# google/deepconsensus

Measured on AMD Instinct MI355X. Metric: zmw_per_sec, higher is better.
Workload: dtype bf16; 1 GPU; global_batch=16384, seq_len=100, windows_per_zmw=150, parallelism=dp1, native_kernels=True, hipgraph=True

## Files before the change

deepconsensus_amd/models/runner.py:

```python
from __future__ import annotations

import copy
import math
from typing import List, Optional, Tuple

import torch

from deepconsensus_amd import ops as dc_ops
from deepconsensus_amd.calibration.calibration import (
    parse_calibration_string,
)
from deepconsensus_amd.models.config import Params
from deepconsensus_amd.models.model import (
    EncoderOnlyLearnedValuesTransformer,
    get_model,
)
from deepconsensus_amd.utils import constants
from deepconsensus_amd.utils import trace


def build_gather_tables(model: EncoderOnlyLearnedValuesTransformer):
    (bi, pwi, ipi, sti, ci, bqi, sni) = model.indices

    def scaled(emb):
        t = emb.table.detach().float() * math.sqrt(emb.width)
        t = t.clone()
        t[0].zero_()
        return t.to(torch.bfloat16)

    tables = {
        "bases": scaled(model.bases_embedding),
        "pw": scaled(model.pw_embedding),
        "ip": scaled(model.ip_embedding),
        "strand": scaled(model.strand_embedding),
        "sn": scaled(model.sn_embedding),
    }
    if model.use_ccs_bq:
        tables["ccs_bq"] = scaled(model.ccs_bq_embedding)

    order = ["bases", "pw", "ip", "strand", "sn"]
    if model.use_ccs_bq:
        order.append("ccs_bq")
    flat_parts, table_base = [], {}
    off = 0
    for name in order:
        t = tables[name]
        table_base[name] = off
        flat = t.reshape(-1)
        pad = (-flat.numel()) % 8
        if pad:
            flat = torch.cat([flat, flat.new_zeros(pad)])
        flat_parts.append(flat)
        off += flat.numel()
    table_flat = torch.cat(flat_parts).contiguous()

    plan: List[Tuple[str, int]] = []
    plan += [("bases", 0)] * (bi[1] - bi[0])
    plan += [("pw", 0)] * (pwi[1] - pwi[0])
    plan += [("ip", 0)] * (ipi[1] - ipi[0])
    plan += [("strand", 0)] * (sti[1] - sti[0])
    plan += [("bases", 0)] * (ci[1] - ci[0])
    if model.use_ccs_bq:
        plan += [("ccs_bq", 1)]
    plan += [("sn", 0)] * (sni[1] - sni[0])

    row_shift = torch.tensor([s for _, s in plan], dtype=torch.int32)
    row_vocab = torch.tensor(
        [tables[n].shape[0] for n, _ in plan], dtype=torch.int32
    )

    cols: List[Tuple[int, int, int]] = []
    for r, (name, _) in enumerate(plan):
        w = tables[name].shape[1]
        base = table_base[name]
        for j in range(w):
            cols.append((r, base, w))
    concat = len(cols)
    assert concat % 8 == 0, f"concat width {concat} not 8-aligned"
    nchunk = concat // 8
    chunk_cnt = torch.zeros(nchunk, dtype=torch.int32)
    chunk_entries = torch.zeros(nchunk * 4, 4, dtype=torch.int32)
    for c in range(nchunk):
        entries = []
        j = c * 8
        while j < (c + 1) * 8:
            r, base, w = cols[j]
            entries.append((r, base, w))
            j += w
        assert len(entries) <= 4, "chunk spans >4 table rows"
        if len(entries) == 1:
            assert entries[0][2] == 8, (
                f"chunk {c}: single entry must be width 8, got "
                f"{entries[0][2]} (row layout misaligned)"
            )
        else:
            assert all(w == 2 for _, _, w in entries), (
                f"chunk {c}: multi-entry chunk must be all width-2 "
                f"entries, got {[w for _, _, w in entries]}"
            )
        chunk_cnt[c] = len(entries)
        for k, (r, base, w) in enumerate(entries):
            chunk_entries[c * 4 + k] = torch.tensor([r, base, w, 0])
    return table_flat, row_shift, row_vocab, chunk_cnt, chunk_entries.reshape(-1)


_CONDENSE_WIDTHS = (560, 568, 872, 880)


def condense_image_stride(k: int) -> Optional[int]:
    if k not in _CONDENSE_WIDTHS:
        return None
    return 16 * (-(-k // 16)) + 8


def build_condense_image(weight: torch.Tensor) -> torch.Tensor:
    n, k = weight.shape
    ws = condense_image_stride(k)
    if ws is None:
        raise ValueError(
            f"fused_condense supports widths {_CONDENSE_WIDTHS}, got {k}"
        )
    npad = -(-n // 64) * 64
    img = torch.zeros(npad, ws, dtype=torch.bfloat16)
    img[:n, :k] = weight.detach().to(torch.bfloat16)
    return img.contiguous()


def fused_condense_enabled(k: int, value: Optional[str]) -> bool:
    if value == "0":
        return False
    if value == "wide":
        return condense_image_stride(k) is not None
    return k == 560


class InferenceRunner:

    def __init__(
        self,
        params: Params,
        model: Optional[torch.nn.Module] = None,
        device: Optional[str] = None,
        calibration: str = "skip",
        max_qual: int = constants.MAX_QUAL,
    ):
        self.params = params
        if device is None:
            device = "cuda" if torch.cuda.is_available() else "cpu"
        self.device = torch.device(device)
        self.calib = parse_calibration_string(calibration)
        self.max_qual = max_qual
        if model is None:
            model = get_model(params)
        model.eval()
        self.model = model

        self.native = (
            self.device.type == "cuda"
            and isinstance(model, EncoderOnlyLearnedValuesTransformer)
            and model.condense
        )
        if self.device.type == "cuda":
            self.ext = dc_ops.get_ext(required=self.native)
        else:
            self.ext = None

        self.model = model.to(self.device)
        if self.native:
            self._prepare_native(model)

    def _prepare_native(self, model) -> None:
        dev, bf16 = self.device, torch.bfloat16
        tf, rs, rv, cc, ce = build_gather_tables(model)
        self.table_flat = tf.to(dev)
        self.row_shift = rs.to(dev)
        self.row_vocab = rv.to(dev)
        self.chunk_cnt = cc.to(dev)
        self.chunk_entries = ce.to(dev)
        self.win = model.params.get("attn_win_size")
        self.num_heads = model.params["num_heads"]
        self.cond_wt = (
            model.condenser.weight.detach().t().contiguous().to(bf16).to(dev)
        )
        self.pos = (
            model.pos_encoding.to(bf16).to(dev)
            if model.add_pos_encoding
            else None
        )
        import os as _os

        self.cond_img = None
        self.pos_f32 = None
        cw = model.condenser.weight.detach()
        if fused_condense_enabled(
            cw.shape[1], _os.environ.get("DC_FUSED_CONDENSE")
        ):
            self.cond_img = build_condense_image(cw).to(dev)
            if model.add_pos_encoding:
                self.pos_f32 = (
                    model.pos_encoding.detach().float().contiguous().to(dev)
                )
        self.fused_embed = _os.environ.get("DC_FUSED_EMBED") != "0"
        self.rezero_fast = all(
            l.attn_wrap.rezero and l.ffn_wrap.rezero for l in model.layers
        ) and self.win is not None
        if self.rezero_fast:
            self.layer_w = []
            for l in model.layers:
                wq = l.attn.q_proj.weight.detach()
                wk = l.attn.k_proj.weight.detach()
                wv = l.attn.v_proj.weight.detach()
                wqkv_t = (
                    torch.cat([wq, wk, wv], 0).t().contiguous().to(bf16).to(dev)
                )
                self.layer_w.append(
                    dict(
                        wqkv_t=wqkv_t,
                        wout_t=l.attn.out_proj.weight.detach()
                        .t().contiguous().to(bf16).to(dev),
                        w1_t=l.ffn.filter_layer.weight.detach()
                        .t().contiguous().to(bf16).to(dev),
                        b1=l.ffn.filter_layer.bias.detach().to(bf16).to(dev),
                        w2_t=l.ffn.output_layer.weight.detach()
                        .t().contiguous().to(bf16).to(dev),
                        b2=l.ffn.output_layer.bias.detach().to(bf16).to(dev),
                        alpha_attn=float(l.attn_wrap.alpha.detach()),
                        alpha_ffn=float(l.ffn_wrap.alpha.detach()),
                    )
                )
            for lw in self.layer_w:
                lw["wout_t_a"] = lw["wout_t"] * lw["alpha_attn"]
                lw["w2_t_a"] = lw["w2_t"] * lw["alpha_ffn"]
                lw["b2_a"] = lw["b2"] * lw["alpha_ffn"]
            import os as _os

            self.ffn_fused_ok = (
                model.params["hidden_size"] == 280
                and model.params["filter_size"] == 2048
                and _os.environ.get("DC_FUSED_FFN") != "0"
            )
            self.ffn_v2 = _os.environ.get("DC_FFN_V2", "1") != "0"
            self.ffn_v3 = _os.environ.get("DC_FFN_V3", "1") != "0"
            self.ffn_v5 = _os.environ.get("DC_FFN_V5", "1") != "0"

            if self.ffn_fused_ok:
                for i, l in enumerate(model.layers):
                    lw = self.layer_w[i]
                    wq = l.attn.q_proj.weight.detach().float()
                    wk = l.attn.k_proj.weight.detach().float()
                    wv = l.attn.v_proj.weight.detach().float()
                    wqkv = torch.cat([wq, wk, wv], 0)
                    wqkv_pad = torch.zeros(896, 296)
                    wqkv_pad[:840, :280] = wqkv
                    lw["wqkv_pad"] = wqkv_pad.to(bf16).contiguous().to(dev)
                    wo = l.attn.out_proj.weight.detach().float()
                    wout_pad = torch.zeros(320, 296)
                    wout_pad[:280, :280] = wo
                    lw["wout_pad"] = wout_pad.to(bf16).contiguous().to(dev)
                    w1 = l.ffn.filter_layer.weight.detach().float()
                    w1p = torch.zeros(2048, 288)
                    w1p[:, :280] = w1
                    lw["w1_pad"] = w1p.to(bf16).contiguous().to(dev)
                    lw["b1_f32"] = (
                        l.ffn.filter_layer.bias.detach().float().to(dev)
                    )
                    w2 = l.ffn.output_layer.weight.detach().float()
                    w2p = torch.zeros(320, 2048)
                    w2p[:280] = w2
                    lw["w2_pad"] = w2p.to(bf16).contiguous().to(dev)
                    b2p = torch.zeros(320)
                    b2p[:280] = l.ffn.output_layer.bias.detach().float()
                    lw["b2_f32"] = b2p.to(dev)
                    w1v2 = torch.zeros(2048, 296)
                    w1v2[:, :280] = w1
                    w1v2[:, 287] = l.ffn.filter_layer.bias.detach().float()
                    lw["w1_v2"] = w1v2.to(bf16).contiguous().to(dev)
            self._addmm_act = hasattr(torch, "_addmm_activation")
            if self._addmm_act:
                try:
                    torch._addmm_activation(
                        torch.zeros(4, device=dev, dtype=bf16),
                        torch.zeros(2, 4, device=dev, dtype=bf16),
                        torch.zeros(4, 4, device=dev, dtype=bf16),
                    )
                except Exception:
                    self._addmm_act = False
        else:
            layers = copy.deepcopy(model.layers).to(bf16)
            for m in layers.modules():
                if isinstance(m, torch.nn.LayerNorm):
                    m.float()
            self.layers_bf16 = layers.to(dev)
        self.ln_gamma = model.output_norm.weight.detach().float().to(dev)
        self.ln_beta = model.output_norm.bias.detach().float().to(dev)
        self.w_head = model.fc1.weight.detach().float().contiguous().to(dev)
        self.b_head = model.fc1.bias.detach().float().to(dev)

    def _attn(self, qkv: torch.Tensor) -> torch.Tensor:
        b, l, w = qkv.shape
        d = w // (3 * self.num_heads)
        if d == 140 and 32 <= l <= 104 and 1 <= self.win <= 12:
            return self.ext.banded_attn_mfma(
                qkv, self.num_heads, self.win, d ** -0.5
            )
        return self.ext.banded_attn(qkv, self.num_heads, self.win)

    @torch.no_grad()
    def encode_native(self, rows: torch.Tensor) -> torch.Tensor:
        rows = rows.contiguous()
        b, _, l = rows.shape
        gather_args = (
            rows, self.table_flat, self.row_shift, self.row_vocab,
            self.chunk_cnt, self.chunk_entries,
        )
        if self.cond_img is not None:
            h = self.cond_wt.shape[1]
            pos = (
                self.pos_f32
                if self.pos_f32 is not None
                else torch.empty(0, dtype=torch.float32, device=rows.device)
            )
            if self.fused_embed:
                with trace.range("K2_K3_embed_condense"):
                    x = self.ext.fused_embed_condense(
                        *gather_args, self.cond_img, pos, h
                    )
            else:
                with trace.range("K2_embed_gather"):
                    emb = self.ext.embed_gather(*gather_args)
                with trace.range("K3_condenser"):
                    x = self.ext.fused_condense(
                        emb.reshape(b * l, -1), self.cond_img, pos, h, l
                    )
            x = x.view(b, l, -1)
        else:
            with trace.range("K2_embed_gather"):
                emb = self.ext.embed_gather(*gather_args)
            with trace.range("K3_condenser"):
                x = emb.reshape(b * l, -1) @ self.cond_wt
            x = x.view(b, l, -1)
            if self.pos is not None:
                x = x + self.pos[:l]
        if self.rezero_fast:
            h = x.shape[-1]
            flat = x.reshape(b * l, h)
            empty = flat.new_empty(0)
            for lw in self.layer_w:
                with trace.range("K5_qkv_proj"):
                    if self.ffn_fused_ok:
                        qkv = self.ext.fused_linear(
                            flat, lw["wqkv_pad"], empty, empty, 840,
                            False, 0.0
                        ).view(b, l, -1)
                    else:
                        qkv = (flat @ lw["wqkv_t"]).view(b, l, -1)
                with trace.range("K6_banded_attn"):
                    a = self._attn(qkv)
                if self.ffn_fused_ok:
                    with trace.range("K7_out_proj"):
                        flat = self.ext.fused_linear(
                            a.view(b * l, h), lw["wout_pad"], empty, flat,
                            280, False, lw["alpha_attn"],
                        )
                    with trace.range("K9_fused_ffn"):
                        if self.ffn_v5:
                            flat = self.ext.fused_ffn_v5(
                                flat, lw["w1_v2"], lw["w2_pad"],
                                lw["b2_f32"], lw["alpha_ffn"],
                            )
                        elif self.ffn_v3:
                            flat = self.ext.fused_ffn_v3(
                                flat, lw["w1_v2"], lw["w2_pad"],
                                lw["b2_f32"], lw["alpha_ffn"],
                            )
                        elif self.ffn_v2:
                            flat = self.ext.fused_ffn_v2(
                                flat, lw["w1_v2"], lw["w2_pad"],
                                lw["b2_f32"], lw["alpha_ffn"],
                            )
                        else:
                            flat = self.ext.fused_ffn(
                                flat, lw["w1_pad"], lw["b1_f32"],
                                lw["w2_pad"], lw["b2_f32"],
                                lw["alpha_ffn"],
                            )
                    continue
                flat = torch.addmm(flat, a.view(b * l, h), lw["wout_t_a"])
                if self._addmm_act:
                    ff = torch._addmm_activation(lw["b1"], flat, lw["w1_t"])
                    flat = torch.addmm(flat, ff, lw["w2_t_a"]).add_(lw["b2_a"])
                else:
                    ff = torch.addmm(lw["b1"], flat, lw["w1_t"]).relu_()
                    flat = torch.addmm(flat, ff, lw["w2_t_a"]).add_(lw["b2_a"])
            x = flat.view(b, l, h)
        else:
            for layer in self.layers_bf16:
                x, _ = layer(x, training=False)
        return x

    @torch.no_grad()
    def forward_windows_graphed(self, host_rows: torch.Tensor):
        if not self.native:
            return self.forward_windows(host_rows)
        shape = tuple(host_rows.shape)
        if getattr(self, "_graph_shape", None) != shape:
            try:
                g_in = torch.empty(
                    shape, dtype=host_rows.dtype, device=self.device
                )
                side = torch.cuda.Stream()
                side.wait_stream(torch.cuda.current_stream())
                with torch.cuda.stream(side):
                    for _ in range(2):
                        self.forward_windows(g_in)
                torch.cuda.current_stream().wait_stream(side)
                torch.cuda.synchronize()
                graph = torch.cuda.CUDAGraph()
                with torch.cuda.graph(graph):
                    g_bases, g_quals = self.forward_windows(g_in)
                torch.cuda.synchronize()
                self._graph = graph
                self._graph_in = g_in
                self._graph_out = (g_bases, g_quals)
                self._graph_shape = shape
            except Exception:
                self._graph_shape = None
                self._graph = None
                return self.forward_windows(host_rows)
        self._graph_in.copy_(host_rows, non_blocking=True)
        self._graph.replay()
        return self._graph_out

    @torch.no_grad()
    def forward_windows(
        self, rows: torch.Tensor, want_probs: bool = False
    ):
        rows = rows.to(self.device, non_blocking=True)
        if self.native:
            x = self.encode_native(rows)
            with trace.range("K10_K12_ln_head_qv"):
                out = self.ext.fused_ln_head_qv(
                x.reshape(-1, x.shape[-1]),
                self.ln_gamma,
                self.ln_beta,
                self.w_head,
                self.b_head,
                float(self.calib.threshold) if self.calib.enabled else -1.0,
                float(self.calib.w) if self.calib.enabled else 1.0,
                float(self.calib.b) if self.calib.enabled else 0.0,
                float(self.max_qual),
                want_probs,
            )
            b, l = rows.shape[0], rows.shape[2]
            bases = out[0].view(b, l)
            quals = out[1].view(b, l)
            if want_probs:
                return bases, quals, out[2].view(b, l, 5)
            return bases, quals
        probs = self.model(rows)
        return self.probs_to_calls(probs, want_probs)

    def probs_to_calls(self, probs: torch.Tensor, want_probs: bool = False):
        pmax, bases = probs.max(dim=-1)
        ep = (1.0 - pmax).clamp_min(1e-12)
        q = -10.0 * torch.log10(ep)
        if self.calib.enabled:
            if self.calib.threshold == 0:
                q = q * self.calib.w + self.calib.b
            else:
                mask = q > self.calib.threshold
                q = torch.where(mask, q * self.calib.w + self.calib.b, q)
        q = q.clamp_max(self.max_qual)
        q = torch.round(q).clamp_min(0)
        bases = bases.to(torch.uint8)
        quals = q.to(torch.uint8)
        if want_probs:
            return bases, quals, probs
        return bases, quals
```

deepconsensus_amd/ops/build.py:

```python
from __future__ import annotations

import os
import shutil

_OPS_DIR = os.path.dirname(os.path.abspath(__file__))
_BUILD_DIR = os.path.join(_OPS_DIR, "_build")
_SRCS = [
    os.path.join(_OPS_DIR, "hip", "dc_kernels.hip"),
    os.path.join(_OPS_DIR, "hip", "banded_attn.hip"),
    os.path.join(_OPS_DIR, "hip", "banded_attn_mfma.hip"),
    os.path.join(_OPS_DIR, "hip", "embed_gather.hip"),
    os.path.join(_OPS_DIR, "hip", "fused_ffn.hip"),
    os.path.join(_OPS_DIR, "hip", "alignment_dp.hip"),
    os.path.join(_OPS_DIR, "hip", "fused_linear.hip"),
    os.path.join(_OPS_DIR, "hip", "fused_ffn_glds.hip"),
    os.path.join(_OPS_DIR, "hip", "fused_ffn_v3.hip"),
    os.path.join(_OPS_DIR, "hip", "embed_grad.hip"),
    os.path.join(_OPS_DIR, "hip", "alignment_metric.hip"),
    os.path.join(_OPS_DIR, "hip", "ffn_ablate.hip"),
    os.path.join(_OPS_DIR, "hip", "banded_attn_train.hip"),
    os.path.join(_OPS_DIR, "hip", "banded_attn_bwd_mfma.hip"),
    os.path.join(_OPS_DIR, "hip", "fused_condense.hip"),
    os.path.join(_OPS_DIR, "hip", "fused_embed_condense.hip"),
    os.path.join(_OPS_DIR, "hip", "ffn_train.hip"),
    os.path.join(_OPS_DIR, "hip", "resid_dropout.hip"),
    os.path.join(_OPS_DIR, "hip", "stitch_compact.hip"),
    os.path.join(_OPS_DIR, "hip", "window_featurize.hip"),
    os.path.join(_OPS_DIR, "hip", "passthrough_fill.hip"),
    os.path.join(_OPS_DIR, "hip", "subread_space.hip"),
    os.path.join(_OPS_DIR, "hip", "fused_ffn_v5.hip"),
    os.path.join(_OPS_DIR, "hip", "alignment_calib.hip"),
    os.path.join(_OPS_DIR, "hip", "cigar_expand.hip"),
]
EXT_NAME = "dc_hip_kernels"


_SPACING_SRC = os.path.join(
    os.path.dirname(_OPS_DIR), "preprocess", "_spacing_cpp.cpp"
)


def build_spacing(verbose: bool = False):
    os.makedirs(_BUILD_DIR, exist_ok=True)
    from torch.utils.cpp_extension import load

    return load(
        name="_spacing",
        sources=[_SPACING_SRC],
        build_directory=_BUILD_DIR,
        extra_cflags=["-O3"],
        verbose=verbose,
    )


def build(verbose: bool = False):
    os.environ.setdefault("PYTORCH_ROCM_ARCH", "gfx950")
    os.makedirs(_BUILD_DIR, exist_ok=True)
    from torch.utils.cpp_extension import load

    build_spacing(verbose=verbose)
    module = load(
        name=EXT_NAME,
        sources=_SRCS,
        build_directory=_BUILD_DIR,
        extra_cuda_cflags=["-O3", "--offload-arch=gfx950"],
        verbose=verbose,
    )
    return module


def build_asan(verbose: bool = False):
    os.environ["PYTORCH_ROCM_ARCH"] = "gfx950:xnack+"
    build_dir = os.path.join(_OPS_DIR, "_build_asan")
    os.makedirs(build_dir, exist_ok=True)
    from torch.utils.cpp_extension import load

    flags = ["-O2", "-fsanitize=address", "-shared-libsan"]
    module = load(
        name=EXT_NAME + "_asan",
        sources=_SRCS,
        build_directory=build_dir,
        extra_cuda_cflags=flags,
        extra_ldflags=[],
        verbose=verbose,
    )
    return module


def clean():
    if os.path.isdir(_BUILD_DIR):
        shutil.rmtree(_BUILD_DIR)


if __name__ == "__main__":
    build(verbose=True)
    print("built", EXT_NAME, "in", _BUILD_DIR)
```

deepconsensus_amd/ops/hip/dc_kernels.hip:

```cpp

#ifndef DC_SAN_MAIN
#include <torch/extension.h>
#include <ATen/hip/HIPContext.h>
#endif
#include <hip/hip_runtime.h>
#include <hip/hip_bf16.h>

#define DC_CHECK(x, msg) TORCH_CHECK(x, msg)

using bf16 = __hip_bfloat16;

namespace {

template <typename T, int NS = 8>
__global__ __launch_bounds__(256) void fused_ln_head_qv_kernel(
    const T* __restrict__ x, const float* __restrict__ gamma,
    const float* __restrict__ beta, const float* __restrict__ w_head,
    const float* __restrict__ b_head, uint8_t* __restrict__ bases_out,
    uint8_t* __restrict__ quals_out, float* __restrict__ probs_out,
    int N, int H, float cal_threshold, float cal_w, float cal_b,
    float max_qual) {
  const int wave_in_block = threadIdx.x >> 6;
  const int lane = threadIdx.x & 63;

  float g[NS], bt[NS], wh[5][NS];
#pragma unroll
  for (int j = 0; j < NS; ++j) {
    const int d = lane + 64 * j;
    g[j] = 0.f;
    bt[j] = 0.f;
#pragma unroll
    for (int k = 0; k < 5; ++k) wh[k][j] = 0.f;
    if (d < H) {
      g[j] = gamma[d];
      bt[j] = beta[d];
#pragma unroll
      for (int k = 0; k < 5; ++k) wh[k][j] = w_head[k * H + d];
    }
  }

  const int stride = gridDim.x * 4;
  int n = blockIdx.x * 4 + wave_in_block;
  T xr[NS];
  if (n < N) {
    const T* xi = x + (size_t)n * H;
#pragma unroll
    for (int j = 0; j < NS; ++j) {
      const int d = lane + 64 * j;
      if (d < H) xr[j] = xi[d];
    }
  }
  for (; n < N; n += stride) {
  float sum = 0.f;
  float xv[NS];
#pragma unroll
  for (int j = 0; j < NS; ++j) {
    if (lane + 64 * j < H) {
      float v;
      if constexpr (std::is_same_v<T, bf16>) v = __bfloat162float(xr[j]);
      else v = xr[j];
      xv[j] = v;
      sum += v;
    }
  }
  if (n + stride < N) {
    const T* xi = x + (size_t)(n + stride) * H;
#pragma unroll
    for (int j = 0; j < NS; ++j) {
      const int d = lane + 64 * j;
      if (d < H) xr[j] = xi[d];
    }
  }
#pragma unroll
  for (int off = 32; off > 0; off >>= 1) sum += __shfl_xor(sum, off, 64);
  const float mean = sum / H;
  float sq = 0.f;
#pragma unroll
  for (int j = 0; j < NS; ++j) {
    if (lane + 64 * j < H) {
      const float dv = xv[j] - mean;
      sq += dv * dv;
    }
  }
#pragma unroll
  for (int off = 32; off > 0; off >>= 1) sq += __shfl_xor(sq, off, 64);
  const float var = sq / H;
  const float rstd = rsqrtf(var + 1e-6f);

  float logit[5];
#pragma unroll
  for (int k = 0; k < 5; ++k) logit[k] = 0.f;
#pragma unroll
  for (int j = 0; j < NS; ++j) {
    if (lane + 64 * j < H) {
      const float normed = (xv[j] - mean) * rstd * g[j] + bt[j];
#pragma unroll
      for (int k = 0; k < 5; ++k) logit[k] += normed * wh[k][j];
    }
  }
#pragma unroll
  for (int off = 32; off > 0; off >>= 1) {
#pragma unroll
    for (int k = 0; k < 5; ++k) logit[k] += __shfl_xor(logit[k], off, 64);
  }

  if (lane == 0) {
    float mx = -1e30f;
#pragma unroll
    for (int k = 0; k < 5; ++k) {
      logit[k] += b_head[k];
      mx = fmaxf(mx, logit[k]);
    }
    float denom = 0.f;
    float ex[5];
#pragma unroll
    for (int k = 0; k < 5; ++k) {
      ex[k] = __expf(logit[k] - mx);
      denom += ex[k];
    }
    int arg = 0;
    float pmax = 0.f;
#pragma unroll
    for (int k = 0; k < 5; ++k) {
      const float p = ex[k] / denom;
      if (probs_out != nullptr) probs_out[(size_t)n * 5 + k] = p;
      if (p > pmax) { pmax = p; arg = k; }
    }
    float ep = 1.f - pmax;
    float q = (ep <= 0.f) ? 1e9f : -10.f * log10f(ep);
    if (cal_threshold == 0.f || q > cal_threshold) q = q * cal_w + cal_b;
    q = fminf(q, max_qual);
    q = nearbyintf(q);
    q = fmaxf(q, 0.f);
    bases_out[n] = (uint8_t)arg;
    quals_out[n] = (uint8_t)q;
  }
  }
}

}

#ifndef DC_SAN_MAIN

std::vector<at::Tensor> fused_ln_head_qv(
    at::Tensor x, at::Tensor gamma, at::Tensor beta, at::Tensor w_head,
    at::Tensor b_head, double cal_threshold, double cal_w, double cal_b,
    double max_qual, bool want_probs) {
  DC_CHECK(x.is_cuda() && x.dim() >= 2, "x must be a device matrix");
  auto xc = x.contiguous();
  const int H = xc.size(-1);
  const int N = xc.numel() / H;
  DC_CHECK(H <= 512, "H must be <= 512");
  auto opts = xc.options();
  auto bases = at::empty({N}, opts.dtype(at::kByte));
  auto quals = at::empty({N}, opts.dtype(at::kByte));
  at::Tensor probs;
  float* probs_ptr = nullptr;
  if (want_probs) {
    probs = at::empty({N, 5}, opts.dtype(at::kFloat));
    probs_ptr = probs.data_ptr<float>();
  }
  dim3 grid(std::min((N + 3) / 4, 2048));
  dim3 block(256);
  hipStream_t stream = at::hip::getCurrentHIPStream();
  auto gc = gamma.contiguous(), bc = beta.contiguous();
  auto wc = w_head.contiguous(), bhc = b_head.contiguous();
  auto launch = [&](auto tag) {
    using T = decltype(tag);
    auto go = [&](auto kern) {
      hipLaunchKernelGGL(kern, grid, block, 0, stream,
                         reinterpret_cast<const T*>(xc.data_ptr()),
                         gc.data_ptr<float>(), bc.data_ptr<float>(),
                         wc.data_ptr<float>(), bhc.data_ptr<float>(),
                         bases.data_ptr<uint8_t>(), quals.data_ptr<uint8_t>(),
                         probs_ptr, N, H, (float)cal_threshold, (float)cal_w,
                         (float)cal_b, (float)max_qual);
    };
    if (H <= 128) go(fused_ln_head_qv_kernel<T, 2>);
    else if (H <= 320) go(fused_ln_head_qv_kernel<T, 5>);
    else go(fused_ln_head_qv_kernel<T, 8>);
  };
  if (xc.dtype() == at::kBFloat16) {
    launch(bf16{});
  } else {
    DC_CHECK(xc.dtype() == at::kFloat, "x must be bf16 or fp32");
    launch(float{});
  }
  if (want_probs) return {bases, quals, probs};
  return {bases, quals};
}

at::Tensor banded_attn(at::Tensor qkv, int64_t H, int64_t win);
at::Tensor banded_attn_mfma(at::Tensor qkv, int64_t H, int64_t win,
                            double scale);
at::Tensor embed_gather(at::Tensor rows, at::Tensor table_flat,
                        at::Tensor row_shift, at::Tensor row_vocab,
                        at::Tensor chunk_cnt, at::Tensor chunk_entries);
at::Tensor fused_ffn(at::Tensor x, at::Tensor w1, at::Tensor b1,
                     at::Tensor w2, at::Tensor b2, double alpha);
at::Tensor fused_ffn_v2(at::Tensor x, at::Tensor w1, at::Tensor w2,
                        at::Tensor b2, double alpha);
at::Tensor fused_ffn_v3(at::Tensor x, at::Tensor w1, at::Tensor w2,
                        at::Tensor b2, double alpha);
at::Tensor fused_ffn_v5(at::Tensor x, at::Tensor w1, at::Tensor w2,
                        at::Tensor b2, double alpha, int64_t max_blocks);
void embed_grad(at::Tensor rows, at::Tensor grad_out, at::Tensor row_shift,
                at::Tensor row_vocab, at::Tensor row_tbase,
                at::Tensor row_width, at::Tensor row_col,
                at::Tensor row_scale, at::Tensor grad_tables);
at::Tensor fused_linear(at::Tensor x, at::Tensor w, at::Tensor bias,
                        at::Tensor resid, int64_t n_out, bool relu,
                        double alpha);
std::vector<at::Tensor> alignment_dp_fwd(at::Tensor subs, at::Tensor ins,
                                         at::Tensor seq_lens, double del_cost,
                                         double reg, int64_t width);
std::vector<at::Tensor> alignment_dp_bwd(at::Tensor grad_out,
                                         at::Tensor weights,
                                         at::Tensor seq_lens, int64_t m,
                                         int64_t n, int64_t width);
std::vector<at::Tensor> alignment_metric_counts(
    at::Tensor yt, at::Tensor yp, at::Tensor yt_len, at::Tensor yp_len,
    double ms, double mp, double go, double ge);
std::vector<at::Tensor> alignment_calib(
    at::Tensor label, at::Tensor bases, at::Tensor quals,
    double ms, double mp, double go, double ge);
at::Tensor ffn_ablate(at::Tensor x, at::Tensor w1, at::Tensor w2,
                      at::Tensor b2, double alpha, int64_t mode);
std::vector<at::Tensor> banded_attn_train_fwd(
    at::Tensor q, at::Tensor k, at::Tensor v, at::Tensor mask,
    int64_t win, double p_drop);
std::vector<at::Tensor> banded_attn_train_bwd(
    at::Tensor q, at::Tensor k, at::Tensor v, at::Tensor p,
    at::Tensor mask, at::Tensor dout, int64_t win, double p_drop);
std::vector<at::Tensor> banded_attn_mfma_train_fwd(
    at::Tensor qkv, int64_t H, int64_t win, double scale,
    at::Tensor drop_mask, double p_drop);
at::Tensor banded_attn_train_bwd2(
    at::Tensor qkv, at::Tensor p, at::Tensor mask, at::Tensor dout,
    int64_t H, int64_t win, double p_drop);
at::Tensor banded_attn_bwd_mfma(
    at::Tensor qkv, at::Tensor p, at::Tensor mask, at::Tensor dout,
    int64_t H, int64_t win, double p_drop);
at::Tensor fused_condense(at::Tensor x, at::Tensor w, at::Tensor pos,
                          int64_t n_out, int64_t seq_len);
at::Tensor fused_embed_condense(at::Tensor rows, at::Tensor table_flat,
                                at::Tensor row_shift, at::Tensor row_vocab,
                                at::Tensor chunk_cnt,
                                at::Tensor chunk_entries, at::Tensor w,
                                at::Tensor pos, int64_t n_out);
std::vector<at::Tensor> ffn_train_fwd(at::Tensor x, at::Tensor w1,
                                      at::Tensor w2, at::Tensor b2,
                                      double p_drop, int64_t seed);
std::vector<at::Tensor> ffn_train_dgrad(at::Tensor dy, at::Tensor hd,
                                        at::Tensor w2t, at::Tensor w1t,
                                        double p_drop);
std::vector<at::Tensor> ffn_train_dgrad_nomask(at::Tensor dy, at::Tensor hd,
                                               at::Tensor w2t,
                                               at::Tensor w1t,
                                               double p_drop);
at::Tensor resid_drop_fwd(at::Tensor x, at::Tensor y, double alpha,
                          double p_drop, int64_t seed);
std::vector<at::Tensor> resid_drop_bwd(at::Tensor dout, at::Tensor y,
                                       double alpha, double p_drop,
                                       int64_t seed);
std::vector<at::Tensor> stitch_compact(at::Tensor bases, at::Tensor quals,
                                       at::Tensor seg_off,
                                       at::Tensor seg_len);
int64_t stitch_compact_into(at::Tensor bases, at::Tensor quals,
                            at::Tensor seg_off, at::Tensor seg_len,
                            at::Tensor seq_out, at::Tensor qual_out,
                            at::Tensor seg_kept, at::Tensor out_off);
at::Tensor window_featurize(at::Tensor sub, at::Tensor ccs,
                            at::Tensor ccs_bq, at::Tensor zmw_tab,
                            at::Tensor win_tab, int64_t R, int64_t L,
                            int64_t max_passes, bool use_ccs_bq);
void window_featurize_into(at::Tensor sub, at::Tensor ccs,
                           at::Tensor ccs_bq, at::Tensor zmw_tab,
                           at::Tensor win_tab, at::Tensor out,
                           int64_t max_passes, bool use_ccs_bq);
void passthrough_fill_into(at::Tensor ccs, at::Tensor ccs_q,
                           at::Tensor zmw_tab, at::Tensor pt_tab,
                           at::Tensor qual_lut, at::Tensor bases_out,
                           at::Tensor quals_out);
void subread_space_into(at::Tensor src, at::Tensor ins_max,
                        at::Tensor sp_tab, at::Tensor read_tab,
                        at::Tensor zmw_tab, at::Tensor col_ref,
                        at::Tensor sub, at::Tensor ccs, at::Tensor ccs_q,
                        at::Tensor ccs_bq, bool use_ccs_bq);
int64_t subread_space_tile();
void cigar_expand_into(at::Tensor raw, at::Tensor op_tab, at::Tensor xr_tab,
                       at::Tensor src, at::Tensor lut);
int64_t cigar_expand_tile();
int64_t cigar_expand_stage();

PYBIND11_MODULE(TORCH_EXTENSION_NAME, m) {
  m.def("cigar_expand_into", &cigar_expand_into,
        "Device alignment expansion: record operands + op tables -> the "
        "unspaced reads (codes | pw | ip) in the caller-owned src of "
        "subread_space_into; lut is the host uint8 [16] base-id table");
  m.def("cigar_expand_tile", &cigar_expand_tile,
        "Elements per tile of cigar_expand_into");
  m.def("cigar_expand_stage", &cigar_expand_stage,
        "Op rows per LDS stage of cigar_expand_into");
  m.def("subread_space_into", &subread_space_into,
        "Device subread spacing: unspaced reads + ins_max -> caller-owned "
        "zero-filled sub / ccs / ccs_q / ccs_bq planes");
  m.def("subread_space_tile", &subread_space_tile,
        "Scan tile (elements) of subread_space_into");
  m.def("passthrough_fill_into", &passthrough_fill_into,
        "Device CCS passthrough: skipped windows of the packed planes -> "
        "caller-owned base-id and QV rows of the stitch buffer");
  m.def("window_featurize", &window_featurize,
        "Device window featurization: compact ZMW planes + window table "
        "-> int16 [N, R, L] model input");
  m.def("window_featurize_into", &window_featurize_into,
        "window_featurize into a caller-owned int16 [N, R, L] tensor");
  m.def("stitch_compact", &stitch_compact,
        "Device window stitching: segmented gap compaction -> (seq_out, "
        "qual_out, seg_kept, out_off)");
  m.def("stitch_compact_into", &stitch_compact_into,
        "stitch_compact into caller-owned output buffers; returns "
        "out_off[S]");
  m.def("fused_condense", &fused_condense,
        "Condenser GEMM [M,560]x[560,N] + fused position-encoding add "
        "(K3+K4)");
  m.def("fused_embed_condense", &fused_embed_condense,
        "Embedding gather inside the condenser GEMM + position-encoding "
        "add (K2+K3+K4): fused_condense(embed_gather(rows)) bit for bit");
  m.def("ffn_train_fwd", &ffn_train_fwd,
        "Training FFN forward: relu + hash dropout in-register, returns "
        "(y, hd)");
  m.def("ffn_train_dgrad", &ffn_train_dgrad,
        "Training FFN dgrad: both transposed GEMMs fused, mask from hd>0, "
        "returns (dx, dh_pre)");
  m.def("ffn_train_dgrad_nomask", &ffn_train_dgrad_nomask,
        "Bisection probe: dgrad without the mask (dh == dy@W2^T)");
  m.def("resid_drop_fwd", &resid_drop_fwd,
        "Fused ReZero residual + hash-dropout forward");
  m.def("resid_drop_bwd", &resid_drop_bwd,
        "Fused residual-dropout backward: (dy, dalpha partials)");
  m.def("fused_ln_head_qv", &fused_ln_head_qv,
        "Fused final LayerNorm + head + softmax + QV (K10+K11+K12)");
  m.def("banded_attn", &banded_attn,
        "Banded multi-head self-attention forward (K5-K7 core, generic)");
  m.def("banded_attn_mfma", &banded_attn_mfma,
        "Banded MHA forward on MFMA (D=140, L<=104)");
  m.def("embed_gather", &embed_gather,
        "Subread-stack embedding gather (K2)");
  m.def("fused_ffn", &fused_ffn,
        "Fused FFN + ReZero residual (K8+K9), hidden tensor LDS-resident");
  m.def("fused_ffn_v2", &fused_ffn_v2,
        "Fused FFN v2: glds-pipelined weights, bias folded into W1");
  m.def("fused_ffn_v3", &fused_ffn_v3,
        "Fused FFN v3: 256-row tiles, register-resident h (swapped B1)");
  m.def("fused_ffn_v5", &fused_ffn_v5,
        "Fused FFN v5: v3 chunk loop in a persistent grid (continuous "
        "weight stream, direct x fragments, 16-B epilogue); max_blocks "
        "caps the grid, 0 = one block per CU",
        pybind11::arg("x"), pybind11::arg("w1"), pybind11::arg("w2"),
        pybind11::arg("b2"), pybind11::arg("alpha"),
        pybind11::arg("max_blocks") = 0);
  m.def("embed_grad", &embed_grad,
        "Fused embedding-stack backward (training, all tables, one pass)");
  m.def("fused_linear", &fused_linear,
        "Fused linear projection (K5/K7): act(xW^T+b)[*alpha+x]");
  m.def("alignment_dp_fwd", &alignment_dp_fwd,
        "Alignment-loss wavefront DP forward (K13)");
  m.def("alignment_dp_bwd", &alignment_dp_bwd,
        "Alignment-loss wavefront DP backward (K13 VJP)");
  m.def("alignment_metric_counts", &alignment_metric_counts,
        "Device AlignmentMetric (K14): affine NW + backtrace counts");
  m.def("alignment_calib", &alignment_calib,
        "Window QV calibration (K14+K15): in-kernel compaction, affine NW "
        "with LDS directions, per-base class + per-QV match/mismatch table");
  m.def("banded_attn_train_fwd", &banded_attn_train_fwd,
        "Training banded attention forward (saves band softmax P)");
  m.def("banded_attn_mfma_train_fwd", &banded_attn_mfma_train_fwd,
        "MFMA training attention forward (serving kernel + band-P save "
        "+ fused dropout)");
  m.def("banded_attn_bwd_mfma", &banded_attn_bwd_mfma,
        "MFMA training attention backward (band_scores/band_apply "
        "primitives; packed dqkv)");
  m.def("banded_attn_train_bwd2", &banded_attn_train_bwd2,
        "Training attention backward v2 (packed qkv layout, 2 blocks/"
        "CU) -> packed dqkv");
  m.def("banded_attn_train_bwd", &banded_attn_train_bwd,
        "Training banded attention backward (band-local dS -> dq,dk,dv)");
  m.def("ffn_ablate", &ffn_ablate,
        "fused_ffn_v3 ablation probe (0 full, 1 B1-only, 2 B2-only, "
        "3 loads-only) — perf diagnosis");
}

#endif
```

Measured before the change: 2518 ZMWs/sec.

## Fold attention out-projection and residual into the persistent fused FFN kernel

Adds a new kernel that computes a @ Wout^T plus the ReZero residual in a per-tile prologue of the persistent v5 FFN kernel, and builds the FFN's A-fragments directly in registers. Wout chunks are streamed through the existing W1/W2 LDS double buffers and interleaved with the first W1/W2 loads. This removes a separate fused_linear launch and its round trip of the intermediate activation through HBM. The mid tensor is still written and then re-read for the epilogue residual. The prologue adds barriers and register pressure to a kernel launched at one block per CU, and this path is on by default when the v5 FFN is active.

```diff
diff --git a/deepconsensus_amd/models/runner.py b/deepconsensus_amd/models/runner.py
--- a/deepconsensus_amd/models/runner.py
+++ b/deepconsensus_amd/models/runner.py
@@ -242,6 +242,9 @@
             self.ffn_v2 = _os.environ.get("DC_FFN_V2", "1") != "0"
             self.ffn_v3 = _os.environ.get("DC_FFN_V3", "1") != "0"
             self.ffn_v5 = _os.environ.get("DC_FFN_V5", "1") != "0"
+            self.fused_outproj = (
+                _os.environ.get("DC_FUSED_OUTPROJ", "1") != "0"
+            )
 
             if self.ffn_fused_ok:
                 for i, l in enumerate(model.layers):
@@ -356,6 +359,14 @@
                         qkv = (flat @ lw["wqkv_t"]).view(b, l, -1)
                 with trace.range("K6_banded_attn"):
                     a = self._attn(qkv)
+                if self.ffn_fused_ok and self.ffn_v5 and self.fused_outproj:
+                    with trace.range("K7_K9_outproj_ffn"):
+                        flat = self.ext.fused_outproj_ffn(
+                            a.view(b * l, h), flat, lw["wout_pad"],
+                            lw["alpha_attn"], lw["w1_v2"], lw["w2_pad"],
+                            lw["b2_f32"], lw["alpha_ffn"],
+                        )
+                    continue
                 if self.ffn_fused_ok:
                     with trace.range("K7_out_proj"):
                         flat = self.ext.fused_linear(
diff --git a/deepconsensus_amd/ops/build.py b/deepconsensus_amd/ops/build.py
--- a/deepconsensus_amd/ops/build.py
+++ b/deepconsensus_amd/ops/build.py
@@ -31,6 +31,7 @@
     os.path.join(_OPS_DIR, "hip", "fused_ffn_v5.hip"),
     os.path.join(_OPS_DIR, "hip", "alignment_calib.hip"),
     os.path.join(_OPS_DIR, "hip", "cigar_expand.hip"),
+    os.path.join(_OPS_DIR, "hip", "fused_outproj_ffn.hip"),
 ]
 EXT_NAME = "dc_hip_kernels"
 
diff --git a/deepconsensus_amd/ops/hip/dc_kernels.hip b/deepconsensus_amd/ops/hip/dc_kernels.hip
--- a/deepconsensus_amd/ops/hip/dc_kernels.hip
+++ b/deepconsensus_amd/ops/hip/dc_kernels.hip
@@ -204,6 +204,10 @@
                         at::Tensor b2, double alpha);
 at::Tensor fused_ffn_v5(at::Tensor x, at::Tensor w1, at::Tensor w2,
                         at::Tensor b2, double alpha, int64_t max_blocks);
+at::Tensor fused_outproj_ffn(at::Tensor a, at::Tensor resid,
+                             at::Tensor wout, double alpha_attn,
+                             at::Tensor w1, at::Tensor w2, at::Tensor b2,
+                             double alpha_ffn, int64_t max_blocks);
 void embed_grad(at::Tensor rows, at::Tensor grad_out, at::Tensor row_shift,
                 at::Tensor row_vocab, at::Tensor row_tbase,
                 at::Tensor row_width, at::Tensor row_col,
@@ -360,6 +364,16 @@
         pybind11::arg("x"), pybind11::arg("w1"), pybind11::arg("w2"),
         pybind11::arg("b2"), pybind11::arg("alpha"),
         pybind11::arg("max_blocks") = 0);
+  m.def("fused_outproj_ffn", &fused_outproj_ffn,
+        "Attention out-projection + ReZero residual (K7) folded into the "
+        "persistent FFN (K9): v5 with a per-tile prologue that builds its "
+        "A-fragments from a @ Wout^T; max_blocks caps the grid, 0 = one "
+        "block per CU",
+        pybind11::arg("a"), pybind11::arg("resid"),
+        pybind11::arg("wout_pad"), pybind11::arg("alpha_attn"),
+        pybind11::arg("w1_v2"), pybind11::arg("w2_pad"),
+        pybind11::arg("b2_f32"), pybind11::arg("alpha_ffn"),
+        pybind11::arg("max_blocks") = 0);
   m.def("embed_grad", &embed_grad,
         "Fused embedding-stack backward (training, all tables, one pass)");
   m.def("fused_linear", &fused_linear,
diff --git a/deepconsensus_amd/ops/hip/fused_outproj_ffn.hip b/deepconsensus_amd/ops/hip/fused_outproj_ffn.hip
--- /dev/null
+++ b/deepconsensus_amd/ops/hip/fused_outproj_ffn.hip
@@ -0,0 +1,348 @@
+
+#ifndef DC_SAN_MAIN
+#include <torch/extension.h>
+#include <ATen/hip/HIPContext.h>
+#endif
+#include <hip/hip_runtime.h>
+#include "ffn_tile.h"
+
+namespace {
+
+typedef float f32x4 __attribute__((ext_vector_type(4)));
+typedef unsigned u32x4 __attribute__((ext_vector_type(4)));
+
+constexpr int EPI_A = W1_ELEMS / 8;
+constexpr int EPI_B = W2_ELEMS / 8;
+constexpr int NQ = NOUT / 8;
+constexpr int EPI_ITERS = (8 * NQ + 63) / 64;
+constexpr int WOUT_HALF_CHUNKS = (32 * K1P * 2 + 1023) / 1024;
+static_assert(NCHUNK % 2 == 0, "chunk 0 must land in buffer 0 every tile");
+static_assert(W2_ELEMS >= W1_ELEMS, "a Wout chunk fits a W2 buffer");
+static_assert(WOUT_HALF_CHUNKS * 512 <= W1_ELEMS, "T8 fits W1[1]");
+static_assert(4 * W1_ELEMS + WOUT_HALF_CHUNKS * 512 <= 320 * K1P,
+              "T8's pieces stay inside wout_pad");
+static_assert(EPI_A * 2 >= 4 * NOUT * 4 && EPI_B * 2 >= 4 * NOUT * 4,
+              "a slice holds 4 fp32 rows");
+static_assert((EPI_A * 2) % 16 == 0 && (EPI_B * 2) % 16 == 0,
+              "slices stay 16-B aligned");
+
+__device__ __forceinline__ float bf16_lo(unsigned w) {
+  return __uint_as_float(w << 16);
+}
+__device__ __forceinline__ float bf16_hi(unsigned w) {
+  return __uint_as_float(w & 0xffff0000u);
+}
+__device__ __forceinline__ unsigned pack_bf16(float lo, float hi) {
+  return (unsigned)__bfloat16_as_ushort(__float2bfloat16(lo)) |
+         ((unsigned)__bfloat16_as_ushort(__float2bfloat16(hi)) << 16);
+}
+
+template <int NCK>
+__device__ __forceinline__ void issue_wout(bf16* smem, const bf16* wout,
+                                           int wave, int chunk,
+                                           int dst_base) {
+  const int ln = lane_recompute();
+  const bf16* src = wout + (size_t)chunk * W1_ELEMS;
+#pragma unroll
+  for (int i = 0; i < 5; ++i) {
+    const int ck = wave + i * 8;
+    if (ck < NCK) {
+      const int dst_off =
+          __builtin_amdgcn_readfirstlane(dst_base + ck * 512);
+      glds16(src + ck * 512 + ln * 8, &smem[dst_off]);
+    }
+  }
+}
+
+template <int F0, int F1>
+__device__ __forceinline__ void load_resid_frags(bf16x8 (&rs)[18],
+                                                 const bf16* rr, bool row_ok,
+                                                 int hi) {
+#pragma unroll
+  for (int f = F0; f < F1; ++f) {
+    rs[f] = bf16x8{};
+    if (row_ok && (f < 17 || hi == 0)) {
+      rs[f] = *reinterpret_cast<const bf16x8*>(rr + 16 * f);
+    }
+  }
+}
+
+template <int T9>
+__device__ __forceinline__ void outproj_tile(const bf16* wbuf,
+                                             const bf16x8 (&aa)[18],
+                                             const bf16x8 (&rs)[18],
+                                             bf16x8 (&af)[18], bf16* mr,
+                                             bool row_ok, float alpha, int c,
+                                             int hi) {
+  f32x16 acc = b1_step(wbuf, aa, T9 & 1, c, hi);
+#pragma unroll
+  for (int r = 0; r < 16; ++r) acc[r] = acc[r] + 0.f;
+  bf16x8 pa[2];
+  t12_repack(acc, pa);
+#pragma unroll
+  for (int s = 0; s < 2; ++s) {
+    const bf16x8 res = rs[2 * T9 + s];
+    bf16x8 v = pa[s];
+#pragma unroll
+    for (int j = 0; j < 8; ++j) {
+      const float rv = (float)res[j];
+      const float vv = (float)v[j];
+      v[j] = (__bf16)(rv + alpha * vv);
+    }
+    if (2 * T9 + s == 17 && hi == 1) {
+      v = __builtin_bit_cast(
+          bf16x8, u32x4{0u, 0u, 0u, row_ok ? 0x3f800000u : 0u});
+    } else if (row_ok) {
+      *reinterpret_cast<bf16x8*>(mr + 16 * (2 * T9 + s)) = v;
+    }
+    af[2 * T9 + s] = v;
+  }
+}
+
+__global__ __launch_bounds__(512, 1) void fused_outproj_ffn_kernel(
+    const bf16* __restrict__ a, const bf16* __restrict__ resid,
+    const bf16* __restrict__ wout, const bf16* __restrict__ w1,
+    const bf16* __restrict__ w2, const float* __restrict__ b2, bf16* mid,
+    bf16* __restrict__ out, int M, float alpha_attn, float alpha, int num_tiles) {
+  __shared__ __attribute__((aligned(16))) bf16 smem[LDS_ELEMS];
+
+  const int wave0 = __builtin_amdgcn_readfirstlane(threadIdx.x >> 6);
+
+  issue_wout<W1_CHUNKS>(smem, wout, wave0, 0, OFF_W1);
+  issue_wout<W1_CHUNKS>(smem, wout, wave0, 1, OFF_W2);
+
+  for (int tile = blockIdx.x; tile < num_tiles; tile += gridDim.x) {
+    const int m0 = tile * BM;
+    const bool has_next = tile + (int)gridDim.x < num_tiles;
+    int wave = wave0;
+    asm volatile("" : "+s"(wave));
+
+    bf16x8 af[18];
+    {
+      const int ln = lane_recompute();
+      const int c = ln & 31;
+      const int hi = ln >> 5;
+      const int row = m0 + 32 * wave + c;
+      const bool row_ok = row < M;
+      const size_t roff = (size_t)(row_ok ? row : 0) * K1 + 8 * hi;
+      const bf16* rr = resid + roff;
+      bf16* mr = mid + roff;
+
+      bf16x8 aa[18];
+      bf16x8 rs[18];
+      if (row_ok) {
+        const bf16* ar = a + roff;
+#pragma unroll
+        for (int s = 0; s < 17; ++s) {
+          aa[s] = *reinterpret_cast<const bf16x8*>(ar + 16 * s);
+        }
+        aa[17] = bf16x8{};
+        if (hi == 0) aa[17] = *reinterpret_cast<const bf16x8*>(ar + 16 * 17);
+      } else {
+#pragma unroll
+        for (int s = 0; s < 18; ++s) aa[s] = bf16x8{};
+      }
+      load_resid_frags<0, 8>(rs, rr, row_ok, hi);
+
+      asm volatile("s_waitcnt vmcnt(0) lgkmcnt(0)" ::: "memory");
+      __builtin_amdgcn_s_barrier();
+
+      load_resid_frags<8, 12>(rs, rr, row_ok, hi);
+      issue_wout<W1_CHUNKS>(smem, wout, wave, 2, OFF_W1 + W1_ELEMS);
+      issue_wout<W1_CHUNKS>(smem, wout, wave, 3, OFF_W2 + W2_ELEMS);
+      outproj_tile<0>(&smem[OFF_W1], aa, rs, af, mr, row_ok, alpha_attn, c,
+                      hi);
+      outproj_tile<1>(&smem[OFF_W1], aa, rs, af, mr, row_ok, alpha_attn, c,
+                      hi);
+      outproj_tile<2>(&smem[OFF_W2], aa, rs, af, mr, row_ok, alpha_attn, c,
+                      hi);
+      outproj_tile<3>(&smem[OFF_W2], aa, rs, af, mr, row_ok, alpha_attn, c,
+                      hi);
+      asm volatile("s_waitcnt vmcnt(0) lgkmcnt(0)" ::: "memory");
+      __builtin_amdgcn_s_barrier();
+
+      load_resid_frags<12, 16>(rs, rr, row_ok, hi);
+      issue_w1(smem, w1, wave, 0, 0);
+      outproj_tile<4>(&smem[OFF_W1 + W1_ELEMS], aa, rs, af, mr, row_ok,
+                      alpha_attn, c, hi);
+      outproj_tile<5>(&smem[OFF_W1 + W1_ELEMS], aa, rs, af, mr, row_ok,
+                      alpha_attn, c, hi);
+      asm volatile("s_waitcnt vmcnt(0) lgkmcnt(0)" ::: "memory");
+      __builtin_amdgcn_s_barrier();
+
+      load_resid_frags<16, 18>(rs, rr, row_ok, hi);
+      issue_wout<WOUT_HALF_CHUNKS>(smem, wout, wave, 4, OFF_W1 + W1_ELEMS);
+      issue_w2(smem, w2, wave, 0, 0);
+      outproj_tile<6>(&smem[OFF_W2 + W2_ELEMS], aa, rs, af, mr, row_ok,
+                      alpha_attn, c, hi);
+      outproj_tile<7>(&smem[OFF_W2 + W2_ELEMS], aa, rs, af, mr, row_ok,
+                      alpha_attn, c, hi);
+      asm volatile("s_waitcnt vmcnt(0) lgkmcnt(0)" ::: "memory");
+      __builtin_amdgcn_s_barrier();
+
+      outproj_tile<8>(&smem[OFF_W1 + W1_ELEMS], aa, rs, af, mr, row_ok,
+                      alpha_attn, c, hi);
+      asm volatile("s_waitcnt vmcnt(0) lgkmcnt(0)" ::: "memory");
+      __builtin_amdgcn_s_barrier();
+    }
+
+    f32x16 oacc[9] = {};
+
+    for (int chunk = 0; chunk < NCHUNK; ++chunk) {
+      const int ln = lane_recompute();
+      const int c = ln & 31;
+      const int hi = ln >> 5;
+      const int buf = chunk & 1;
+      if (chunk + 1 < NCHUNK) {
+        issue_w1(smem, w1, wave, chunk + 1, buf ^ 1);
+        issue_w2(smem, w2, wave, chunk + 1, buf ^ 1);
+      } else if (has_next) {
+        issue_wout<W1_CHUNKS>(smem, wout, wave, 0, OFF_W1);
+        issue_wout<W1_CHUNKS>(smem, wout, wave, 1, OFF_W2);
+      }
+      const bf16* w1buf = &smem[OFF_W1 + buf * W1_ELEMS];
+      const bf16* w2buf = &smem[OFF_W2 + buf * W2_ELEMS];
+
+#pragma unroll
+      for (int t = 0; t < 2; ++t) {
+        const f32x16 acc = b1_step(w1buf, af, t, c, hi);
+        f32x16 st;
+#pragma unroll
+        for (int r = 0; r < 16; ++r) st[r] = acc[r] > 0.f ? acc[r] : 0.f;
+        bf16x8 pa[2];
+        t12_repack(st, pa);
+        b2_step(w2buf, pa, oacc, t, c, hi);
+      }
+
+      asm volatile("s_waitcnt vmcnt(0) lgkmcnt(0)" ::: "memory");
+      __builtin_amdgcn_s_barrier();
+    }
+
+    {
+      const int lne = lane_recompute();
+      const int ce = lne & 31;
+      const int hie = lne >> 5;
+      float* slice_a =
+          reinterpret_cast<float*>(&smem[OFF_W1 + W1_ELEMS + wave * EPI_A]);
+      float* slice_b =
+          reinterpret_cast<float*>(&smem[OFF_W2 + W2_ELEMS + wave * EPI_B]);
+      float* slice_w = hie ? slice_b : slice_a;
+      float bias[9];
+#pragma unroll
+      for (int ct = 0; ct < 9; ++ct) bias[ct] = b2[min(32 * ct + ce, NOUT - 1)];
+      u32x4 rv[4][EPI_ITERS];
+      auto load_resid = [&](int g) {
+#pragma unroll
+        for (int it = 0; it < EPI_ITERS; ++it) {
+          const int idx = min(it * 64 + lne, 8 * NQ - 1);
+          const int row = min(m0 + 32 * wave + 8 * g + idx / NQ, M - 1);
+          rv[g][it] = *reinterpret_cast<const u32x4*>(
+              mid + (size_t)row * K1 + 8 * (idx % NQ));
+        }
+      };
+      load_resid(0);
+      load_resid(1);
+      load_resid(2);
+#pragma unroll
+      for (int g = 0; g < 4; ++g) {
+#pragma unroll
+        for (int ct = 0; ct < 9; ++ct) {
+          const int col = 32 * ct + ce;
+          if (col < NOUT) {
+#pragma unroll
+            for (int j = 0; j < 4; ++j) {
+              slice_w[j * NOUT + col] = oacc[ct][4 * g + j] + bias[ct];
+            }
+          }
+        }
+        if (g == 0) load_resid(3);
+        asm volatile("s_waitcnt lgkmcnt(0)" ::: "memory");
+#pragma unroll
+        for (int it = 0; it < EPI_ITERS; ++it) {
+          const int idx = it * 64 + lne;
+          const int rl = idx / NQ, q = idx % NQ;
+          const int row = m0 + 32 * wave + 8 * g + rl;
+          if (idx < 8 * NQ && row < M) {
+            const float* src =
+                (rl < 4 ? slice_a + rl * NOUT : slice_b + (rl - 4) * NOUT) +
+                8 * q;
+            const f32x4 t0 = *reinterpret_cast<const f32x4*>(src);
+            const f32x4 t1 = *reinterpret_cast<const f32x4*>(src + 4);
+            const u32x4 r = rv[g][it];
+            u32x4 ov;
+            ov.x = pack_bf16(bf16_lo(r.x) + alpha * t0.x,
+                             bf16_hi(r.x) + alpha * t0.y);
+            ov.y = pack_bf16(bf16_lo(r.y) + alpha * t0.z,
+                             bf16_hi(r.y) + alpha * t0.w);
+            ov.z = pack_bf16(bf16_lo(r.z) + alpha * t1.x,
+                             bf16_hi(r.z) + alpha * t1.y);
+            ov.w = pack_bf16(bf16_lo(r.w) + alpha * t1.z,
+                             bf16_hi(r.w) + alpha * t1.w);
+            *reinterpret_cast<u32x4*>(out + (size_t)row * K1 + 8 * q) = ov;
+          }
+        }
+        asm volatile("s_waitcnt lgkmcnt(0)" ::: "memory");
+      }
+    }
+  }
+}
+
+}
+
+#ifndef DC_SAN_MAIN
+
+at::Tensor fused_outproj_ffn(at::Tensor a, at::Tensor resid,
+                             at::Tensor wout, double alpha_attn,
+                             at::Tensor w1, at::Tensor w2, at::Tensor b2,
+                             double alpha_ffn, int64_t max_blocks) {
+  TORCH_CHECK(a.is_cuda() && a.dtype() == at::kBFloat16,
+              "a must be bf16 on device");
+  TORCH_CHECK(resid.is_cuda() && resid.dtype() == at::kBFloat16,
+              "resid must be bf16 on device");
+  auto ac = a.contiguous();
+  auto rc = resid.contiguous();
+  const int K = ac.size(-1);
+  const int M = ac.numel() / K;
+  TORCH_CHECK(K == K1, "fused_outproj_ffn requires width 280");
+  TORCH_CHECK(rc.numel() == ac.numel(), "resid must match a");
+  TORCH_CHECK(wout.is_cuda() && wout.dtype() == at::kBFloat16 &&
+                  wout.dim() == 2 && wout.is_contiguous() &&
+                  wout.size(0) == 320 && wout.size(1) == K1P,
+              "wout must be contiguous bf16 [320, 296]");
+  TORCH_CHECK(w1.is_cuda() && w1.dtype() == at::kBFloat16 &&
+                  w1.is_contiguous() && w1.dim() == 2 &&
+                  w1.size(0) == NHID && w1.size(1) == K1P,
+              "w1 must be [2048, 296] with b1 folded into column 287");
+  TORCH_CHECK(w2.is_cuda() && w2.dtype() == at::kBFloat16 &&
+                  w2.is_contiguous() && w2.dim() == 2 &&
+                  w2.size(0) == 320 && w2.size(1) == NHID,
+              "w2 must be padded [320, 2048]");
+  TORCH_CHECK(b2.numel() >= NOUT, "b2 must cover 280 outputs");
+  TORCH_CHECK(max_blocks >= 0, "max_blocks must be >= 0 (0 = one per CU)");
+  auto b2c = b2.contiguous();
+  TORCH_CHECK(b2c.is_cuda() && b2c.dtype() == at::kFloat, "b2 must be fp32");
+  auto out = at::empty({M, K1}, ac.options());
+  const int num_tiles = (M + BM - 1) / BM;
+  if (num_tiles == 0) return out;
+  auto mid = at::empty({M, K1}, ac.options());
+  const int64_t cap =
+      max_blocks > 0
+          ? max_blocks
+          : at::cuda::getCurrentDeviceProperties()->multiProcessorCount;
+  dim3 grid((unsigned)std::min<int64_t>(num_tiles, cap));
+  dim3 block(512);
+  hipStream_t stream = at::hip::getCurrentHIPStream();
+  hipLaunchKernelGGL(fused_outproj_ffn_kernel, grid, block, 0, stream,
+                     reinterpret_cast<bf16*>(ac.data_ptr()),
+                     reinterpret_cast<bf16*>(rc.data_ptr()),
+                     reinterpret_cast<bf16*>(wout.data_ptr()),
+                     reinterpret_cast<bf16*>(w1.data_ptr()),
+                     reinterpret_cast<bf16*>(w2.data_ptr()),
+                     b2c.data_ptr<float>(),
+                     reinterpret_cast<bf16*>(mid.data_ptr()),
+                     reinterpret_cast<bf16*>(out.data_ptr()), M,
+                     (float)alpha_attn, (float)alpha_ffn, num_tiles);
+  return out;
+}
+
+#endif
```

After: 2605 ZMWs/sec (median of 6 runs). 3.5% higher.
